# konstantineder/montecarlo-risk-engine

Hardware: AMD Instinct MI355X
Metric: path-steps/sec at 1M paths x 250 steps; PV/CVA rel-error vs CPU ref (higher is better)
Workload: dtype f64

## Files before the change

### montecarlo-risk-engine_amd/csrc/kf_lean.hip

```cpp
#include <cstdlib>
#include <map>
#include <utility>

#include "kf_common.h"

namespace {

template <int NSLOT, int PPL>
__device__ __forceinline__ void lean_date_cva(const FastDateCvaLds* __restrict__ rp, const double (&reg)[PPL][2 * NSLOT], double (&cva)[PPL],
                                              const double* __restrict__ etab)
{
    const mcx_expq_coef ec = mcx_expq_load(mcx_region_zero());
    const FastDateCvaLds r = *rp;
    double xe[2 * PPL], ev[2 * PPL];
#pragma unroll
    for (int q = 0; q < PPL; ++q) {
        xe[2 * q] = fma(r.m_s1, reg[q][FDC_S_REG], fma(r.m_n1, reg[q][FDC_NI_REG], r.m_c0));
        xe[2 * q + 1] = fma(r.c_c1, reg[q][FDC_C_REG], r.c_c0);
    }
    mcx_exp_tab_n<2 * PPL>(xe, ev, etab, ec);
#pragma unroll
    for (int q = 0; q < PPL; ++q) {
        const double x = fma(r.x_d, reg[q][FDC_X_REG], r.x_a);
        double p = 0.0;
        p += fma(fma(r.row0[2], x, r.row0[1]), x, r.row0[0]);
        p += fma(fma(r.row1[2], x, r.row1[1]), x, r.row1[0]);
        const double w = r.m_b * ev[2 * q];
        const double cs = fma(r.c_b, ev[2 * q + 1], r.c_a);
        cva[q] = fma(fmax(p, 0.0), w * (1.0 - cs), cva[q]);
    }
}

#define MCX_LEAN_WAVES 4
template <int NSLOT, int NZ, bool INJECT, int SIG, int PPL, bool SIMULATE, int DK = 0>
__global__ __launch_bounds__(MCX_BLOCK, MCX_LEAN_WAVES) void kf_lean(const FusedArgs)
{
    static_assert(DK == 0 || (SIG == SIG_VAS_CIR_E && SIMULATE && !INJECT), "the cva-date kernel simulates the Vasicek + CIR++ signature");
    constexpr int NREG = 2 * NSLOT;
    constexpr int TILE = MCX_BLOCK * PPL;
    extern __shared__ double lds[];
    KArgs& a0 = kargs_region(0);
    const int n_rec = a0.n_rec;
    const int64_t n = a0.k1.n;
    for (int q = threadIdx.x; q < 9 * n_rec; q += MCX_BLOCK) lds[q] = 0.0;
    FastDateCvaLds* const dlds = (FastDateCvaLds*)(lds + ((9 * n_rec + 1) & ~1));
    if constexpr (DK == 1) {
        const FastDateCva* __restrict__ dc = a0.cva_dates;
        const double* __restrict__ cf = a0.coeffs;
        const int n_dates = a0.n_dates;
        for (int q = threadIdx.x; q < 16 * n_dates; q += MCX_BLOCK) {
            const int t = q >> 4, e = q & 15;
            double v;
            if (e < FDC_HEAD) {
                v = ((const double*)(dc + t))[e];
            } else {
                const int off = e < FDC_HEAD + 3 ? dc[t].coeff_off0 : dc[t].coeff_off1;
                v = off >= 0 ? cf[off + (e - FDC_HEAD) % 3] : 0.0;
            }
            ((double*)dlds)[q] = v;
        }
    }
    constexpr int BMB = SIG == SIG_VAS_CIR_E ? 10 : 7;
    constexpr int BM = (INJECT || !SIMULATE) ? 0 : MCX_BM_LDS_DOUBLES_B(BMB);
    __shared__ double tab_lds[BM + MCX_EXP_LDS_DOUBLES];
    const double* tab = nullptr;
    const double* etab = tab_lds + BM;
    mcx_exp_tab_load(tab_lds + BM);
    if (BM) { mcx_bm_load<BMB>(tab_lds); tab = tab_lds; }
    __syncthreads();
    const int64_t tiles = (n + TILE - 1) / TILE;
    double n_block = 0.0;

    for (int64_t tile = blockIdx.x; tile < tiles; tile += gridDim.x) {
        const bool first_tile = tile == (int64_t)blockIdx.x;
        int64_t i[PPL];
        bool live[PPL];
        uint64_t path[PPL];
        double reg[PPL][NREG];
        double cfs[PPL], cva[PPL];
        int est[PPL];
        int n_init, n_steps;
        {
            KArgs& a = kargs_region(mcx_region_zero());
            const auto& k = a.k1;
#pragma unroll
            for (int q = 0; q < PPL; ++q) {
                const int64_t i_raw = tile * TILE + q * MCX_BLOCK + threadIdx.x;
                live[q] = i_raw < n;
                i[q] = live[q] ? i_raw : n - 1;
                path[q] = k.path_offset + (uint64_t)i[q];
                sim_init_state<NSLOT, SIG>(k, reg[q]);
                cfs[q] = 0.0; cva[q] = 0.0;
                est[q] = a.init_state[0];
            }
            const int64_t rest = n - tile * TILE;
            n_block += (double)(rest < TILE ? rest : TILE);
            n_init = k.n_initial_store; n_steps = k.n_steps;
        }
        if (SIMULATE) {
        int step = 0, t_init = 0;
#pragma unroll 1
        while (true) {
            const bool init = t_init < n_init;
            if (!init && step >= n_steps) break;
            int st = init ? t_init : -1;
            t_init += init ? 1 : 0;
            {
                const int zr0 = mcx_region_zero();
                const auto& k = kargs_region(zr0).k1;
                const uint64_t seed = k.seed;
                const mcx_bm_coef bc = mcx_bm_coef_load(zr0);
                const mcx_bm_vconst vc = mcx_bm_vconst_make<BMB>(bc);
#pragma unroll 1
                while (st < 0 && step < n_steps) {
                    if constexpr (SIG == SIG_GENERIC) {
#pragma unroll
                        for (int q = 0; q < PPL; ++q) sim_substep<NSLOT, NZ, INJECT, SIG, BMB, true>(k, step, path[q], i[q], reg[q], tab, seed, bc, &vc);
                        st = ldk(&k.steps[step].store_idx);
                    } else {
                        double zz[PPL][NZ], uu[PPL];
                        bool rare = false;
                        const StepData<NSLOT, NZ> sdat = sim_step_load<NSLOT, NZ, SIG>(k, step);
                        __builtin_amdgcn_sched_barrier(0);
                        if constexpr (INJECT) {
#pragma unroll
                            for (int q = 0; q < PPL; ++q) sim_draw<NZ, true, SIG, BMB>(k, step, path[q], i[q], zz[q], uu[q], tab, seed, bc, &vc);
                        } else {
                            uint32_t st_q[PPL];
#pragma unroll
                            for (int q = 0; q < PPL; ++q) st_q[q] = (uint32_t)step;
                            rare = sim_draw_n<PPL, NZ, SIG, BMB>(k, st_q, path, zz, uu, tab, seed, bc, vc);
                        }
                        if (!INJECT && __builtin_expect(__any(rare), 0)) {
#pragma unroll
                            for (int q = 0; q < PPL; ++q) sim_draw<NZ, false, SIG, BMB, true>(k, step, path[q], i[q], zz[q], uu[q], tab, seed, bc, &vc);
                        }
#pragma unroll
                        for (int q = 0; q < PPL; ++q) st = sim_apply_loaded<NSLOT, NZ, SIG, true>(k, sdat, reg[q], zz[q], uu[q]);
                    }
                    ++step;
                }
            }
            if (st >= 0) {
                if constexpr (DK == 1) lean_date_cva<NSLOT, PPL>(dlds + st, reg, cva, etab);
                else lean_date<NSLOT, SIG, PPL, true>(st, i, live, first_tile, lds, reg, cfs, cva, est, etab);
            }
        }
        } else {
            auto load_row = [&](int t, double (&dst)[PPL][NREG]) {
                const auto& k = kargs_region(0).k1;
                const int D = k.n_state;
#pragma unroll
                for (int q = 0; q < PPL; ++q)
#pragma unroll
                    for (int sl = 0; sl < NSLOT; ++sl) {
                        const bool bs = sig_kind(SIG, sl) >= 0 ? sig_is_bs(SIG, sl) : (k.slots[sl].kind == MCX_MODEL_BS);
                        const int c = k.slots[sl].state_off;
                        dst[q][2 * sl] = k.paths[((int64_t)t * D + c) * k.ld + i[q]];
                        dst[q][2 * sl + 1] = bs ? 0.0 : k.paths[((int64_t)t * D + c + 1) * k.ld + i[q]];
                    }
            };
            const int n_dates = kargs_region(0).n_dates;
            double bufb[PPL][NREG];
            load_row(0, reg);
            load_row(n_dates > 1 ? 1 : 0, bufb);
#pragma unroll 1
            for (int t = 0; t < n_dates; t += 2) {
                lean_date<NSLOT, SIG, PPL, false>(t, i, live, first_tile, lds, reg, cfs, cva, est, etab);
                if (t + 2 < n_dates) load_row(t + 2, reg);
                if (t + 1 < n_dates) {
                    lean_date<NSLOT, SIG, PPL, false>(t + 1, i, live, first_tile, lds, bufb, cfs, cva, est, etab);
                    if (t + 3 < n_dates) load_row(t + 3, bufb);
                }
            }
        }
        {
            KArgs& a = kargs_region(mcx_region_zero());
#pragma unroll
            for (int q = 0; q < PPL; ++q) if (a.cfs && live[q]) a.cfs[i[q]] = cfs[q];
            if (a.rec_pv[0] >= 0) lean_record<PPL>(cfs, live, a.rec_pv[0], n_rec, first_tile, lds);
            if (a.rec_cva[0] >= 0) {
                const double lgd = a.lgd[0];
                double cc[PPL];
#pragma unroll
                for (int q = 0; q < PPL; ++q) cc[q] = cva[q] * lgd;
                lean_record<PPL>(cc, live, a.rec_cva[0], n_rec, first_tile, lds);
            }
        }
    }
    __syncthreads();
    for (int r = threadIdx.x; r < n_rec; r += MCX_BLOCK) {
        double s1 = 0.0, s2 = 0.0;
        for (int w = 0; w < 4; ++w) { s1 += lds[n_rec + (w * n_rec + r) * 2]; s2 += lds[n_rec + (w * n_rec + r) * 2 + 1]; }
        double* dst = a0.partials + ((int64_t)blockIdx.x * n_rec + r) * 4;
        dst[0] = n_block; dst[1] = lds[r]; dst[2] = s1; dst[3] = s2;
    }
}

template <int NSLOT, int NZ, int SIG, int PPL>
int launch_lean_shape(const FusedArgs& a, int n_cu, bool inject, bool simulate, hipStream_t s)
{
    const int64_t tiles = (a.k1.n + MCX_BLOCK * PPL - 1) / (MCX_BLOCK * PPL);
    const size_t lds = sizeof(double) * (size_t)((9 * a.n_rec + 1) & ~1);
    const size_t lds_cva = lds + sizeof(FastDateCvaLds) * (size_t)a.n_dates;
    auto residency = [&](auto kernel, size_t bytes) {
        thread_local std::map<std::pair<const void*, size_t>, int> cache;
        const auto key = std::make_pair((const void*)kernel, bytes);
        auto it = cache.find(key);
        if (it == cache.end()) {
            int per_cu = 0;
            if (hipOccupancyMaxActiveBlocksPerMultiprocessor(&per_cu, kernel, MCX_BLOCK, bytes) != hipSuccess || per_cu < 1) per_cu = 1;
            it = cache.emplace(key, per_cu < MCX_LEAN_WAVES ? per_cu : MCX_LEAN_WAVES).first;
        }
        return (int64_t)it->second * n_cu;
    };
    auto sized = [&](int64_t resident) {
        if (tiles <= resident) return (int)tiles;
        const int64_t per = (tiles + resident - 1) / resident;
        return (int)((tiles + per - 1) / per);
    };
    int grid;
    if (!simulate) {
        auto kern = kf_lean<NSLOT, NZ, false, SIG, PPL, false>;
        grid = sized(residency(kern, lds));
        hipLaunchKernelGGL(kern, dim3(grid), dim3(MCX_BLOCK), lds, s, a);
    } else if (inject) {
        auto kern = kf_lean<NSLOT, NZ, true, SIG, PPL, true>;
        grid = sized(residency(kern, lds));
        hipLaunchKernelGGL(kern, dim3(grid), dim3(MCX_BLOCK), lds, s, a);
    } else {
        auto kern = kf_lean<NSLOT, NZ, false, SIG, PPL, true>;
        const int64_t resident = residency(kern, lds);
        if constexpr (SIG == SIG_VAS_CIR_E) {
            auto kern_cva = kf_lean<NSLOT, NZ, false, SIG, PPL, true, 1>;
            if (a.cva_dates && residency(kern_cva, lds_cva) >= resident) {
                grid = sized(resident);
                hipLaunchKernelGGL(kern_cva, dim3(grid), dim3(MCX_BLOCK), lds_cva, s, a);
                return grid;
            }
        }
        grid = sized(resident);
        hipLaunchKernelGGL(kern, dim3(grid), dim3(MCX_BLOCK), lds, s, a);
    }
    return grid;
}

template <int NSLOT, int NZ, int SIG>
void launch_lean(const FusedArgs& a, int n_cu, bool inject, bool simulate, hipStream_t s, int* grid_out)
{
    constexpr int PPL = (SIG == SIG_GENERIC && NSLOT >= 2) ? 1 : 2;
#ifdef MCX_LEAN_AB
    if (simulate && !inject) {
        const char* sh = getenv("MCX_LEAN_SHAPE");
        const int code = sh ? atoi(sh) : 0;
        if (code == 11) { *grid_out = launch_lean_shape<NSLOT, NZ, SIG, 1>(a, n_cu, inject, simulate, s); return; }
        if (code == 21) { *grid_out = launch_lean_shape<NSLOT, NZ, SIG, 2>(a, n_cu, inject, simulate, s); return; }
    }
#endif
    const int64_t full_tiles = (a.k1.n + MCX_BLOCK * PPL - 1) / (MCX_BLOCK * PPL);
    if (PPL == 2 && simulate && !inject && full_tiles < (int64_t)2 * n_cu) {
        *grid_out = launch_lean_shape<NSLOT, NZ, SIG, 1>(a, n_cu, inject, simulate, s);
        return;
    }
    *grid_out = launch_lean_shape<NSLOT, NZ, SIG, PPL>(a, n_cu, inject, simulate, s);
}

}

int mcx_launch_kf_lean(const FusedArgs& a, const mcx_sim_desc& sd, int n_cu, bool inject, bool simulate, hipStream_t s)
{
    int grid = -1;
    switch (mcx_sim_signature(sd)) {
    case SIG_VAS_CIR_E: launch_lean<2, 2, SIG_VAS_CIR_E>(a, n_cu, inject, simulate, s, &grid); break;
#ifndef MCX_LEAN_ONE_SIG
    case SIG_BS_A: launch_lean<1, 1, SIG_BS_A>(a, n_cu, inject, simulate, s, &grid); break;
    case SIG_BS_E: launch_lean<1, 1, SIG_BS_E>(a, n_cu, inject, simulate, s, &grid); break;
    case SIG_HESTON_QE: launch_lean<1, 2, SIG_HESTON_QE>(a, n_cu, inject, simulate, s, &grid); break;
    case SIG_HESTON_E: launch_lean<1, 2, SIG_HESTON_E>(a, n_cu, inject, simulate, s, &grid); break;
    case SIG_VAS_E: launch_lean<1, 1, SIG_VAS_E>(a, n_cu, inject, simulate, s, &grid); break;
    case SIG_VAS_A: launch_lean<1, 1, SIG_VAS_A>(a, n_cu, inject, simulate, s, &grid); break;
    case SIG_BS_VAS_CIRDET_E: launch_lean<3, 3, SIG_BS_VAS_CIRDET_E>(a, n_cu, inject, simulate, s, &grid); break;
    default:
        switch (sd.n_slots * 16 + sd.n_z) {
        case 1 * 16 + 1: launch_lean<1, 1, SIG_GENERIC>(a, n_cu, inject, simulate, s, &grid); break;
        case 1 * 16 + 2: launch_lean<1, 2, SIG_GENERIC>(a, n_cu, inject, simulate, s, &grid); break;
        case 2 * 16 + 2: launch_lean<2, 2, SIG_GENERIC>(a, n_cu, inject, simulate, s, &grid); break;
        case 3 * 16 + 3: launch_lean<3, 3, SIG_GENERIC>(a, n_cu, inject, simulate, s, &grid); break;
        case 4 * 16 + 4: launch_lean<4, 4, SIG_GENERIC>(a, n_cu, inject, simulate, s, &grid); break;
        default: break;
        }
#else
    default: break;
#endif
    }
    return grid;
}
```

### montecarlo-risk-engine_amd/csrc/mcx_device.h

```cpp
#pragma once
#include "mcx_internal.h"

struct K1Args {
    mcx_slot slots[MCX_MAX_SLOTS];
    double init_state[MCX_MAX_STATE];
    const mcx_step* __restrict__ steps;
    const double* __restrict__ chol;
    const double* __restrict__ aux;
    double* __restrict__ paths;
    const double* __restrict__ inject_z;
    const double* __restrict__ inject_u;
    const double* __restrict__ init_paths;
    int64_t n, ld;
    uint64_t seed, path_offset;
    int32_t scheme, n_steps, n_state, n_initial_store, flags, n_uniform;
};

static inline void mcx_fill_k1_args(const mcx_sim* sim, uint64_t seed, uint64_t path_offset, int64_t n_paths, int64_t ld,
                                    double* d_paths, const double* d_inject_z, const double* d_inject_u, K1Args* a)
{
    const mcx_sim_desc& d = sim->desc;
    memset(a, 0, sizeof(*a));
    for (int s = 0; s < d.n_slots; ++s) a->slots[s] = d.slots[s];
    for (int c = 0; c < d.n_state; ++c) a->init_state[c] = d.init_state[c];
    a->steps = sim->d_steps; a->chol = sim->d_chol; a->aux = sim->d_aux;
    a->paths = d_paths; a->inject_z = d_inject_z; a->inject_u = d_inject_u;
    a->n = n_paths; a->ld = ld; a->seed = seed; a->path_offset = path_offset;
    a->scheme = d.scheme; a->n_steps = d.n_steps; a->n_state = d.n_state; a->n_initial_store = d.n_initial_store;
    a->flags = d.flags; a->n_uniform = d.n_uniform;
}

__device__ __forceinline__ void philox4x32_10(uint32_t c0, uint32_t c1, uint32_t c2, uint32_t c3, uint32_t k0, uint32_t k1,
                                              uint32_t& o0, uint32_t& o1, uint32_t& o2, uint32_t& o3)
{
#pragma unroll
    for (int r = 0; r < 10; ++r) {
        const uint64_t p0 = (uint64_t)0xD2511F53u * c0;
        const uint64_t p1 = (uint64_t)0xCD9E8D57u * c2;
        const uint32_t n0 = __builtin_amdgcn_bitop3_b32((uint32_t)(p1 >> 32), c1, k0, 0x96);
        const uint32_t n2 = __builtin_amdgcn_bitop3_b32((uint32_t)(p0 >> 32), c3, k1, 0x96);
        c1 = (uint32_t)p1;
        c3 = (uint32_t)p0;
        c0 = n0;
        c2 = n2;
        k0 += 0x9E3779B9u;
        k1 += 0xBB67AE85u;
    }
    o0 = c0; o1 = c1; o2 = c2; o3 = c3;
}

__device__ __forceinline__ double u53(uint32_t lo, uint32_t hi, const mcx_bm_vconst* vc = nullptr)
{
    if (vc) return fma((double)hi, vc->s32, fma((double)(lo >> 11), vc->s53, vc->c54));
    return fma((double)hi, 0x1.0p-32, fma((double)(lo >> 11), 0x1.0p-53, 0x1.0p-54));
}

struct DevBridge {
    uint64_t seed, path_offset;
    const double* const* inject;
    int64_t ld;
};

__device__ __forceinline__ double dev_barrier_event(const DevEvent& e, const DevTerm* __restrict__ terms, const double* __restrict__ coeffs,
                                                    const DevBridge* __restrict__ bridge, const double* __restrict__ paths, int64_t D,
                                                    int64_t ld, int64_t i, double num)
{
    const int types = (int)e.aux[3];
    const int t1 = types & 7, t2 = types >> 3;
    const bool with_bridge = e.aux[0] == 5.0;
    double mx = -1.0e300, mn = 1.0e300, keep1 = 1.0, keep2 = 1.0, prev1 = 0.0, prev2 = 0.0;
    double c = 0.0;
    int draw_id = 0;
    DevBridge br = {0, 0, nullptr, 0};
    const double* __restrict__ inj = nullptr;
    if (with_bridge) {
        c = ldk(coeffs + e.coeff_off);
        draw_id = (int)ldk(coeffs + e.coeff_off + 1);
        br = ldk_struct(bridge);
        if (br.inject) inj = br.inject[draw_id];
    }
    AtomCache bc = {-1, -1, 0.0};
    for (int j = e.term_begin; j < e.term_end; ++j) {
        const double s = dev_atom_cached(ldk_struct(&terms[j]).atom, paths, D, ld, i, bc);
        mx = fmax(mx, s); mn = fmin(mn, s);
        if (with_bridge) {
            const double cur1 = mcx_log(s / e.aux[1]), cur2 = t2 ? mcx_log(s / e.aux[2]) : 0.0;
            if (j > e.term_begin) {
                const int k = j - e.term_begin - 1;
                for (int bi = 0; bi < (t2 ? 2 : 1); ++bi) {
                    const double p = mcx_exp(c * (bi ? prev2 * cur2 : prev1 * cur1));
                    double u;
                    if (inj) u = inj[(int64_t)(2 * k + bi) * br.ld + i];
                    else {
                        uint32_t w0, w1, w2, w3;
                        const uint64_t path = br.path_offset + (uint64_t)i;
                        philox4x32_10((uint32_t)path, (uint32_t)(path >> 32), (uint32_t)k, 0x80000000u | (uint32_t)(2 * draw_id + bi),
                                      (uint32_t)br.seed, (uint32_t)(br.seed >> 32), w0, w1, w2, w3);
                        u = u53(w0, w1);
                    }
                    const double hit = fmin(fmax((p - u + 0.05) / 0.1, 0.0), 1.0);
                    if (bi) keep2 *= 1.0 - hit; else keep1 *= 1.0 - hit;
                }
            }
            prev1 = cur1; prev2 = cur2;
        }
    }
    double pay = fmax(e.sign * (dev_atom(e.x, paths, D, ld, i) - e.strike), 0.0) * dev_barrier_ind(t1, e.aux[1], mx, mn);
    if (with_bridge) pay *= (t1 <= 2) ? keep1 : 1.0 - keep1;
    if (t2) {
        pay *= dev_barrier_ind(t2, e.aux[2], mx, mn);
        if (with_bridge) pay *= (t2 <= 2) ? keep2 : 1.0 - keep2;
    }
    return pay / num;
}

template <bool TAB = false, int BMB = 7, bool GUARD = true>
__device__ __forceinline__ bool pair_from_words(uint32_t w0, uint32_t w1, uint32_t w2, uint32_t w3, double& ua, double& z0, double& z1,
                                                const double* __restrict__ tab, const mcx_bm_coef& bc, const mcx_bm_vconst* vc = nullptr)
{
    ua = u53(w0, w1, vc);
    double s, c, r;
    if (TAB) {
        const double r2 = mcx_m2log_tab<BMB>(ua, tab, bc, vc);
        if (!GUARD) r = mcx_sqrt_gp(r2);
        else if (__builtin_expect(__any(w1 == 0xffffffffu), 0)) r = ua < 1.0 ? mcx_sqrt_g(r2) : 0.0;
        else r = mcx_sqrt_gp(r2);
        const int j = (int)(w3 >> (32 - BMB));
        const double ur = u53(w2, w3 & ((1u << (32 - BMB)) - 1u), vc);
        mcx_sincos2pi_tab<BMB>(ur, j, tab, s, c, bc, vc);
    } else {
        r = mcx_sqrt(-2.0 * mcx_log(ua));
        mcx_sincos2pi(u53(w2, w3), s, c);
    }
    z0 = r * c;
    z1 = r * s;
    return w1 == 0xffffffffu;
}

template <bool TAB = false, int BMB = 7, bool GUARD = true>
__device__ __forceinline__ bool draw_pair(uint64_t seed, uint64_t path, uint32_t step, uint32_t draw, double& ua, double& z0, double& z1,
                                          const double* __restrict__ tab, const mcx_bm_coef& bc, const mcx_bm_vconst* vc = nullptr)
{
    uint32_t w0, w1, w2, w3;
    philox4x32_10((uint32_t)path, (uint32_t)(path >> 32), step, draw, (uint32_t)seed, (uint32_t)(seed >> 32), w0, w1, w2, w3);
    return pair_from_words<TAB, BMB, GUARD>(w0, w1, w2, w3, ua, z0, z1, tab, bc, vc);
}

template <bool TAB = false>
__device__ __forceinline__ void draw_pair(uint64_t seed, uint64_t path, uint32_t step, uint32_t draw, double& ua, double& z0, double& z1,
                                          const double* __restrict__ tab = nullptr)
{
    const mcx_bm_coef bc = mcx_bm_coef_load();
    draw_pair<TAB>(seed, path, step, draw, ua, z0, z1, tab, bc);
}

__device__ __forceinline__ double degree_of_truth(double x, bool fuzzy, double eps)
{
    if (!fuzzy) return x > 0.0 ? 1.0 : 0.0;
    const double v = (x + eps) / (2.0 * eps);
    return fmin(fmax(v, 0.0), 1.0);
}

struct AuxPtr {
    const double* __restrict__ p;
    __device__ __forceinline__ double operator[](int i) const { return ldk(p + i); }
    __device__ __forceinline__ mcx_aux_drv drv() const { return ldk_struct((const mcx_aux_drv*)(p + MCX_AUX_C0)); }
};
struct AuxRegs {
    double v[MCX_AUX];
    __device__ __forceinline__ double operator[](int i) const { return v[i]; }
    __device__ __forceinline__ mcx_aux_drv drv() const { mcx_aux_drv d; d.c0 = v[MCX_AUX_C0]; d.c1 = v[MCX_AUX_C1]; d.c2 = v[MCX_AUX_C2]; return d; }
};

template <int KIND, int SCHEME, bool POS = false, class SL, class AUX>
__device__ __forceinline__ void step_slot(const SL& sl, int scheme_rt, int flags, double dt, double sq,
                                          const AUX& aux, double& s0, double& s1, double zc0, double zc1, double u)
{
    const auto* p = sl.p;
    const int scheme = SCHEME >= 0 ? SCHEME : scheme_rt;
    switch (KIND >= 0 ? KIND : sl.kind) {
    case MCX_MODEL_BS:
        if (scheme == MCX_SCHEME_ANALYTICAL) {
            s0 = s0 * mcx_exp(aux[0] + (zc0 - aux[1]));
        } else {
            const mcx_aux_drv dc = aux.drv();
            s0 = fma(s0, fma(dc.c2, zc0, dc.c0), s0);
        }
        break;
    case MCX_MODEL_VASICEK: {
        const double r = s0;
        s1 = s1 + r * dt;
        if (scheme == MCX_SCHEME_ANALYTICAL) s0 = (p[2] + (r - p[2]) * aux[0]) + zc0;
        else {
            const mcx_aux_drv dc = aux.drv();
            s0 = fma(dc.c1, r, s0);
            s0 = fma(dc.c2, zc0, s0);
            s0 = s0 + dc.c0;
        }
        break;
    }
    case MCX_MODEL_HW: {
        const double r = s0;
        s1 = s1 + r * dt;
        if (scheme == MCX_SCHEME_ANALYTICAL) s0 = r * aux[0] + aux[1] + zc0;
        else s0 = r + (aux[0] - p[3] * r) * dt + p[1] * sq * zc0;
        break;
    }
    case MCX_MODEL_CIRPP: {
        const double y = s0;
        const double sy = POS ? mcx_sqrt_gp(y) : mcx_sqrt_g(y);
        const mcx_aux_drv dc = aux.drv();
        s1 = fma(y + aux[0], dt, s1);
        s0 = fma(dc.c1, y, s0);
        s0 = fma(dc.c2 * sy, zc0, s0);
        s0 = s0 + dc.c0;
        s0 = fmax(s0, 1e-12);
        break;
    }
    case MCX_MODEL_CIRPP_DET:
        s1 = s1 + aux[0] * dt;
        s0 = aux[1];
        break;
    case MCX_MODEL_S2F: {
        const double x = s0, y = s1;
        if (scheme == MCX_SCHEME_ANALYTICAL) {
            s0 = x * aux[0] + zc0;
            s1 = y + p[3] * dt + zc1;
        } else {
            s0 = x - p[1] * x * dt + p[2] * sq * zc0;
            s1 = y + p[3] * dt + p[4] * sq * zc1;
        }
        break;
    }
    case MCX_MODEL_HESTON: {
        const double logS = s0, v = s1;
        const double sigma = p[1], rate = p[2], kappa = p[4], theta = p[5];
        if (scheme == MCX_SCHEME_EULER) {
            const double sv = mcx_sqrt(fmax(v, 0.0));
            s0 = logS + (rate - 0.5 * v) * dt + sv * sq * zc0;
            s1 = fmax(v + kappa * (theta - v) * dt + sigma * sv * sq * zc1, 0.0);
        } else {
            const double eps = 1e-12;
            const bool fuzzy = (flags & MCX_FLAG_SMOOTHING) != 0;
            const double m = theta + (v - theta) * aux[0];
            const double s2 = v * aux[6] + aux[7];
            const double omu = fmax(1.0 - u, eps);
            const double d1 = m * m + eps, d5 = m + eps;
            const double d15 = d1 * d5;
            const double ra = mcx_rcp(d15 * omu);
            const double r_omu = ra * d15, ra6 = ra * omu;
            const double r1 = ra6 * d5, r5 = ra6 * d1;
            const double psi = s2 * r1;
            const double d2 = psi + eps, d4 = psi + 1.0;
            const double rb = mcx_rcp(d2 * d4);
            const double invpsi = rb * d4, r4 = rb * d2;
            const double t = fmax(2.0 * invpsi - 1.0, 0.0);
            double root = mcx_sqrt_g(2.0 * invpsi * t);
            root = invpsi < 0.0 ? __builtin_nan("") : root;
            const double b2u = 2.0 * invpsi - 1.0 + root;
            const double b2 = b2u < 0.0 ? 0.0 : b2u;
            const double b = mcx_sqrt_g(b2);
            const double pp = fmin(fmax((psi - 1.0) * r4, 0.0), 1.0 - 1e-6);
            const double beta = (1.0 - pp) * r5;
            const double d3 = 1.0 + b2, d7 = beta + eps;
            const double rc = mcx_rcp(d3 * d7);
            const double a = m * (rc * d7);
            const double v1 = a * (b + zc1) * (b + zc1);
            const double omp = fmax(1.0 - pp, eps);
            const double v_tail = mcx_log(omp * r_omu) * (rc * d3);
            const double v2 = degree_of_truth(u - pp, fuzzy, 0.3) * v_tail;
            const double w = degree_of_truth(psi - 1.5, fuzzy, 0.5);
            const double vn = (1.0 - w) * v1 + w * v2;
            const double var_int = fmax(aux[4] * v + aux[5] * vn, 0.0);
            const double vol = mcx_sqrt_gp(fmax(var_int, eps));
            s0 = logS + rate * dt + aux[1] + aux[2] * v + aux[3] * vn + vol * zc0;
            s1 = vn;
        }
        break;
    }
    default: break;
    }
}


enum { SIG_GENERIC = 0, SIG_VAS_CIR_E = 1, SIG_BS_A = 2, SIG_BS_E = 3, SIG_HESTON_QE = 4, SIG_HESTON_E = 5,
       SIG_VAS_E = 6, SIG_VAS_A = 7, SIG_BS_VAS_CIRDET_E = 8 };

__host__ __device__ constexpr int sig_kind(int sig, int slot)
{
    return sig == SIG_VAS_CIR_E ? (slot == 0 ? MCX_MODEL_VASICEK : MCX_MODEL_CIRPP)
         : (sig == SIG_BS_A || sig == SIG_BS_E) ? MCX_MODEL_BS
         : (sig == SIG_HESTON_QE || sig == SIG_HESTON_E) ? MCX_MODEL_HESTON
         : (sig == SIG_VAS_E || sig == SIG_VAS_A) ? MCX_MODEL_VASICEK
         : sig == SIG_BS_VAS_CIRDET_E ? (slot == 0 ? MCX_MODEL_BS : slot == 1 ? MCX_MODEL_VASICEK : MCX_MODEL_CIRPP_DET)
         : -1;
}
__host__ __device__ constexpr int sig_scheme(int sig)
{
    return (sig == SIG_VAS_CIR_E || sig == SIG_BS_E || sig == SIG_HESTON_E || sig == SIG_VAS_E || sig == SIG_BS_VAS_CIRDET_E) ? MCX_SCHEME_EULER
         : (sig == SIG_BS_A || sig == SIG_VAS_A) ? MCX_SCHEME_ANALYTICAL
         : sig == SIG_HESTON_QE ? MCX_SCHEME_QE : -1;
}
__host__ __device__ constexpr bool sig_is_bs(int sig, int slot) { return sig_kind(sig, slot) == MCX_MODEL_BS; }

static inline int mcx_sim_signature(const mcx_sim_desc& d)
{
    auto k = [&](int s) { return d.slots[s].kind; };
    if (d.n_slots == 2 && k(0) == MCX_MODEL_VASICEK && k(1) == MCX_MODEL_CIRPP && d.scheme == MCX_SCHEME_EULER) return SIG_VAS_CIR_E;
    if (d.n_slots == 3 && k(0) == MCX_MODEL_BS && k(1) == MCX_MODEL_VASICEK && k(2) == MCX_MODEL_CIRPP_DET && d.scheme == MCX_SCHEME_EULER)
        return SIG_BS_VAS_CIRDET_E;
    if (d.n_slots == 1) {
        if (k(0) == MCX_MODEL_BS) return d.scheme == MCX_SCHEME_ANALYTICAL ? SIG_BS_A : d.scheme == MCX_SCHEME_EULER ? SIG_BS_E : SIG_GENERIC;
        if (k(0) == MCX_MODEL_HESTON) return d.scheme == MCX_SCHEME_QE ? SIG_HESTON_QE : d.scheme == MCX_SCHEME_EULER ? SIG_HESTON_E : SIG_GENERIC;
        if (k(0) == MCX_MODEL_VASICEK) return d.scheme == MCX_SCHEME_EULER ? SIG_VAS_E : d.scheme == MCX_SCHEME_ANALYTICAL ? SIG_VAS_A : SIG_GENERIC;
    }
    return SIG_GENERIC;
}

__device__ __forceinline__ AuxPtr aux_of_slot(const double* __restrict__ ax, int s) { return AuxPtr{ax + s * MCX_AUX}; }
template <int NSLOT>
__device__ __forceinline__ const AuxRegs& aux_of_slot(const AuxRegs (&ax)[NSLOT], int s) { return ax[s]; }

template <int NSLOT, int NZ, int SIG, int S, bool POS = false, class KA, class AX>
__device__ __forceinline__ void step_slots(const KA& k, const mcx_step& sp, const AX& ax,
                                           double (&reg)[2 * NSLOT], const double (&zc)[NZ], double u)
{
    if constexpr (S < NSLOT) {
        const double zc0 = (NSLOT == 1) ? zc[0] : zc[S < NZ ? S : 0];
        const double zc1 = (NSLOT == 1 && NZ > 1) ? zc[NZ > 1 ? 1 : 0] : 0.0;
        step_slot<sig_kind(SIG, S), sig_scheme(SIG), POS>(k.slots[S], k.scheme, k.flags | k.slots[S].flags, sp.dt, sp.sqrt_dt,
                                                      aux_of_slot(ax, S), reg[2 * S], reg[2 * S + 1], zc0, zc1, u);
        step_slots<NSLOT, NZ, SIG, S + 1, POS>(k, sp, ax, reg, zc, u);
    }
}

template <int NZ, bool INJECT, int SIG, int BMB = 7, bool GUARD = true, class KA>
__device__ __forceinline__ bool sim_draw(const KA& k, int step, uint64_t path, int64_t i, double (&z)[NZ], double& u,
                                         const double* __restrict__ tab, uint64_t seed, const mcx_bm_coef& bc, const mcx_bm_vconst* vc = nullptr)
{
    u = 0.0;
    bool rare = false;
    if (INJECT) {
#pragma unroll
        for (int j = 0; j < NZ; ++j) z[j] = k.inject_z[((int64_t)step * NZ + j) * k.ld + i];
        if (k.n_uniform) u = k.inject_u[(int64_t)step * k.ld + i];
    } else {
        double ua;
#pragma unroll
        for (int q = 0; q < (NZ + 1) / 2; ++q) {
            double z0, z1;
            rare |= draw_pair<true, BMB, GUARD>(seed, path, (uint32_t)step, (uint32_t)q, ua, z0, z1, tab, bc, vc);
            z[2 * q] = z0;
            if (2 * q + 1 < NZ) z[2 * q + 1] = z1;
        }
        if (sig_scheme(SIG) == MCX_SCHEME_QE || (sig_scheme(SIG) < 0 && k.n_uniform)) {
            double z0, z1;
            draw_pair<false>(seed, path, (uint32_t)step, (uint32_t)((NZ + 1) / 2), u, z0, z1, nullptr, bc);
        }
    }
    return rare;
}

template <int PPL>
__device__ __forceinline__ void philox4x32_10_n(const uint64_t (&path)[PPL], const uint32_t (&step)[PPL], uint32_t draw, uint64_t seed,
                                                uint32_t (&o0)[PPL], uint32_t (&o1)[PPL], uint32_t (&o2)[PPL], uint32_t (&o3)[PPL])
{
    uint32_t c0[PPL], c1[PPL], c2[PPL], c3[PPL];
#pragma unroll
    for (int q = 0; q < PPL; ++q) { c0[q] = (uint32_t)path[q]; c1[q] = (uint32_t)(path[q] >> 32); c2[q] = step[q]; c3[q] = draw; }
    uint32_t k0 = (uint32_t)seed, k1 = (uint32_t)(seed >> 32);
#pragma unroll
    for (int r = 0; r < 10; ++r) {
#pragma unroll
        for (int q = 0; q < PPL; ++q) {
            const uint64_t p0 = (uint64_t)0xD2511F53u * c0[q];
            const uint64_t p1 = (uint64_t)0xCD9E8D57u * c2[q];
            const uint32_t n0 = __builtin_amdgcn_bitop3_b32((uint32_t)(p1 >> 32), c1[q], k0, 0x96);
            const uint32_t n2 = __builtin_amdgcn_bitop3_b32((uint32_t)(p0 >> 32), c3[q], k1, 0x96);
            c1[q] = (uint32_t)p1; c3[q] = (uint32_t)p0; c0[q] = n0; c2[q] = n2;
        }
        k0 += 0x9E3779B9u;
        k1 += 0xBB67AE85u;
    }
#pragma unroll
    for (int q = 0; q < PPL; ++q) { o0[q] = c0[q]; o1[q] = c1[q]; o2[q] = c2[q]; o3[q] = c3[q]; }
}

template <int PPL, int BMB>
__device__ __forceinline__ bool draw_pairs_staged(uint64_t seed, const uint64_t (&path)[PPL], const uint32_t (&step)[PPL], uint32_t draw,
                                                  double (&z0)[PPL], double (&z1)[PPL], const double* __restrict__ tab,
                                                  const mcx_bm_coef& C, const mcx_bm_vconst& vc)
{
    constexpr int N = 1 << BMB, LOG_TERMS = mcx_bm_shape<BMB>::LOG_TERMS;
    uint32_t w0[PPL], w1[PPL], w2[PPL], w3[PPL];
    philox4x32_10_n<PPL>(path, step, draw, seed, w0, w1, w2, w3);
    double m[PPL], ed[PPL], ps[PPL], pc[PPL];
    int e[PPL];
    mcx_d2 tc[PPL], sc[PPL];
#pragma unroll
    for (int q = 0; q < PPL; ++q) {
        const double ua = u53(w0[q], w1[q], &vc);
        m[q] = __builtin_amdgcn_frexp_mant(ua);
        e[q] = __builtin_amdgcn_frexp_exp(ua);
        const int jl = (__double2hiint(m[q]) >> (20 - BMB)) & (N - 1);
        tc[q] = ((const mcx_d2*)tab)[jl];
        sc[q] = ((const mcx_d2*)(tab + 2 * N))[(int)(w3[q] >> (32 - BMB))];
    }
    __builtin_amdgcn_sched_barrier(0);
#pragma unroll
    for (int q = 0; q < PPL; ++q) {
        const double ur = u53(w2[q], w3[q] & ((1u << (32 - BMB)) - 1u), &vc);
        const double d = fma(ur, 6.28318530717958647692, vc.trig_off);
        const double d2 = d * d;
        double qs, qc;
        if constexpr (mcx_bm_shape<BMB>::TRIG_TERMS == 3) {
            qs = fma(fma(vc.sin_head, d2, C.c[7]), d2, C.c[6]);
            qc = fma(fma(vc.cos_head, d2, C.c[10]), d2, C.c[9]);
        } else {
            qs = fma(vc.sin_head, d2, C.c[6]);
            qc = fma(vc.cos_head, d2, C.c[9]);
        }
        ps[q] = fma(d * d2, qs, d);
        pc[q] = fma(d2, qc, 1.0);
        ed[q] = (double)e[q];
    }
    __builtin_amdgcn_sched_barrier(0);
    bool rare = false;
#pragma unroll
    for (int q = 0; q < PPL; ++q) {
        const double s = fma(m[q], tc[q].x, 2.0);
        double p = vc.log_head;
#pragma unroll
        for (int k = LOG_TERMS - 2; k >= 0; --k) p = fma(p, s, C.c[k]);
        const double r2 = fma(ed[q], -2.0 * 6.93147180559945309417e-01, tc[q].y) + fma(s * s, p, s);
        const double r = mcx_sqrt_gp(r2);
        const double sn = fma(sc[q].x, pc[q], sc[q].y * ps[q]);
        const double cs = fma(-sc[q].x, ps[q], sc[q].y * pc[q]);
        z0[q] = r * cs;
        z1[q] = r * sn;
        rare |= w1[q] == 0xffffffffu;
    }
    return rare;
}

template <int PPL, int NZ, int SIG, int BMB, class KA>
__device__ __forceinline__ bool sim_draw_n(const KA& k, const uint32_t (&step)[PPL], const uint64_t (&path)[PPL], double (&z)[PPL][NZ], double (&u)[PPL],
                                           const double* __restrict__ tab, uint64_t seed, const mcx_bm_coef& bc, const mcx_bm_vconst& vc)
{
    bool rare = false;
#pragma unroll
    for (int dq = 0; dq < (NZ + 1) / 2; ++dq) {
        double a[PPL], b[PPL];
        rare |= draw_pairs_staged<PPL, BMB>(seed, path, step, (uint32_t)dq, a, b, tab, bc, vc);
#pragma unroll
        for (int q = 0; q < PPL; ++q) { z[q][2 * dq] = a[q]; if (2 * dq + 1 < NZ) z[q][2 * dq + 1] = b[q]; }
    }
#pragma unroll
    for (int q = 0; q < PPL; ++q) {
        u[q] = 0.0;
        if (sig_scheme(SIG) == MCX_SCHEME_QE || (sig_scheme(SIG) < 0 && k.n_uniform)) {
            double t0, t1;
            draw_pair<false>(seed, path[q], step[q], (uint32_t)((NZ + 1) / 2), u[q], t0, t1, nullptr, bc);
        }
    }
    return rare;
}

template <int NSLOT, int NZ, int SIG, bool POS = false, class KA>
__device__ __forceinline__ int sim_apply(const KA& k, int step, double (&reg)[2 * NSLOT], const double (&z)[NZ], double u)
{
    const mcx_step sp = ldk_struct(&k.steps[step]);
    double zc[NZ];
    constexpr bool UNIT_L00 = sig_scheme(SIG) == MCX_SCHEME_EULER || sig_scheme(SIG) == MCX_SCHEME_QE;
    const double* __restrict__ L = UNIT_L00 ? k.chol : k.chol + (int64_t)sp.chol_idx * NZ * NZ;
#pragma unroll
    for (int r = 0; r < NZ; ++r) {
        double acc = (UNIT_L00 && r == 0) ? z[0] : ldk(L + r * NZ) * z[0];
#pragma unroll
        for (int c = 1; c <= r; ++c) acc = fma(ldk(L + r * NZ + c), z[c], acc);
        zc[r] = acc;
    }
    const double* __restrict__ ax = k.aux + (int64_t)step * NSLOT * MCX_AUX;
    step_slots<NSLOT, NZ, SIG, 0, POS>(k, sp, ax, reg, zc, u);
    return sp.store_idx;
}

template <int NSLOT, int NZ>
struct StepData {
    mcx_step sp;
    double L[NZ * NZ];
    AuxRegs ax[NSLOT];
};
template <int NSLOT, int NZ, int SIG, class KA>
__device__ __forceinline__ StepData<NSLOT, NZ> sim_step_load(const KA& k, int step)
{
    StepData<NSLOT, NZ> d;
    d.sp = ldk_struct(&k.steps[step]);
    constexpr bool UNIT_L00 = sig_scheme(SIG) == MCX_SCHEME_EULER || sig_scheme(SIG) == MCX_SCHEME_QE;
    const double* __restrict__ L = UNIT_L00 ? k.chol : k.chol + (int64_t)d.sp.chol_idx * NZ * NZ;
#pragma unroll
    for (int q = 0; q < NZ * NZ; ++q) d.L[q] = ldk(L + q);
    struct P2 { double v[2]; };
    struct P4 { double v[4]; };
    static_assert(MCX_AUX == 8, "aux row layout");
    const double* __restrict__ ax = k.aux + (int64_t)step * NSLOT * MCX_AUX;
#pragma unroll
    for (int s = 0; s < NSLOT; ++s) {
        const P2 a = ldk_struct((const P2*)(ax + s * MCX_AUX)), b = ldk_struct((const P2*)(ax + s * MCX_AUX + 2));
        const P4 c = ldk_struct((const P4*)(ax + s * MCX_AUX + 4));
        d.ax[s].v[0] = a.v[0]; d.ax[s].v[1] = a.v[1]; d.ax[s].v[2] = b.v[0]; d.ax[s].v[3] = b.v[1];
#pragma unroll
        for (int q = 0; q < 4; ++q) d.ax[s].v[4 + q] = c.v[q];
    }
    return d;
}
template <int NSLOT, int NZ, int SIG, bool POS = false, class KA>
__device__ __forceinline__ int sim_apply_loaded(const KA& k, const StepData<NSLOT, NZ>& d, double (&reg)[2 * NSLOT], const double (&z)[NZ], double u)
{
    double zc[NZ];
    constexpr bool UNIT_L00 = sig_scheme(SIG) == MCX_SCHEME_EULER || sig_scheme(SIG) == MCX_SCHEME_QE;
#pragma unroll
    for (int r = 0; r < NZ; ++r) {
        double acc = (UNIT_L00 && r == 0) ? z[0] : d.L[r * NZ] * z[0];
#pragma unroll
        for (int c = 1; c <= r; ++c) acc = fma(d.L[r * NZ + c], z[c], acc);
        zc[r] = acc;
    }
    step_slots<NSLOT, NZ, SIG, 0, POS>(k, d.sp, d.ax, reg, zc, u);
    return d.sp.store_idx;
}

template <int NSLOT, int NZ, bool INJECT, int SIG, int BMB = 7, bool POS = false, class KA>
__device__ __forceinline__ void sim_substep(const KA& k, int step, uint64_t path, int64_t i, double (&reg)[2 * NSLOT],
                                            const double* __restrict__ tab, uint64_t seed, const mcx_bm_coef& bc, const mcx_bm_vconst* vc = nullptr)
{
    double z[NZ], u;
    sim_draw<NZ, INJECT, SIG, BMB>(k, step, path, i, z, u, tab, seed, bc, vc);
    sim_apply<NSLOT, NZ, SIG, POS>(k, step, reg, z, u);
}

__host__ __device__ constexpr int mcx_kind_state_dim(int kind) { return kind == MCX_MODEL_BS ? 1 : kind == MCX_MODEL_S2F ? 3 : 2; }

template <int NSLOT, int SIG, class KA>
__device__ __forceinline__ void sim_init_state(const KA& k, double (&reg)[2 * NSLOT], int64_t i = 0)
{
    const double* __restrict__ ip = k.init_paths;
#pragma unroll
    for (int s = 0; s < NSLOT; ++s) {
        const int kind = sig_kind(SIG, s) >= 0 ? sig_kind(SIG, s) : k.slots[s].kind;
        const int c = k.slots[s].state_off + (kind == MCX_MODEL_S2F ? 1 : 0);
        if (ip) {
            reg[2 * s] = ip[(int64_t)c * k.ld + i];
            reg[2 * s + 1] = kind == MCX_MODEL_BS ? 0.0 : ip[(int64_t)(c + 1) * k.ld + i];
        } else {
            reg[2 * s] = k.init_state[c];
            reg[2 * s + 1] = kind == MCX_MODEL_BS ? 0.0 : k.init_state[c + 1];
        }
    }
}

template <int NSLOT, int SIG, class KA>
__device__ __forceinline__ void sim_store_state(const KA& k, int t, int64_t i, const double (&reg)[2 * NSLOT],
                                                const double* __restrict__ ax = nullptr)
{
    const int D = k.n_state;
#pragma unroll
    for (int s = 0; s < NSLOT; ++s) {
        const int kind = sig_kind(SIG, s) >= 0 ? sig_kind(SIG, s) : k.slots[s].kind;
        const int c = k.slots[s].state_off;
        if (kind == MCX_MODEL_S2F) {
            const double logF = ax ? ldk(ax + s * MCX_AUX + 1) : k.slots[s].p[6];
            double logS = (logF + reg[2 * s]) + reg[2 * s + 1];
            if (!ax && k.init_paths) logS = k.init_paths[(int64_t)c * k.ld + i];
            k.paths[((int64_t)t * D + c) * k.ld + i] = logS;
            k.paths[((int64_t)t * D + c + 1) * k.ld + i] = reg[2 * s];
            k.paths[((int64_t)t * D + c + 2) * k.ld + i] = reg[2 * s + 1];
            continue;
        }
        k.paths[((int64_t)t * D + c) * k.ld + i] = reg[2 * s];
        if (kind != MCX_MODEL_BS) k.paths[((int64_t)t * D + c + 1) * k.ld + i] = reg[2 * s + 1];
    }
}
```

Baseline: 291.8 billion.

## Specialise Philox first rounds for uniform path high word and stop after last live CVA date

When every path in the launch shares the same upper 32 bits of the path index, a UHI kernel variant is selected. It partly evaluates the first three Philox rounds, using the known zero high counter word and the wave-uniform high bits, which removes a few multiplies and xors per draw. Separately, the CVA-date kernel scans the date table for the last date with nonzero regression coefficients and ends simulation once that date is processed, skipping the remaining steps. This adds template instantiations and host-side selection logic. The early exit assumes dates whose coefficients are all zero contribute nothing to CVA.

```diff
diff --git a/montecarlo-risk-engine_amd/csrc/kf_lean.hip b/montecarlo-risk-engine_amd/csrc/kf_lean.hip
--- a/montecarlo-risk-engine_amd/csrc/kf_lean.hip
+++ b/montecarlo-risk-engine_amd/csrc/kf_lean.hip
@@ -32,10 +32,11 @@
 }
 
 #define MCX_LEAN_WAVES 4
-template <int NSLOT, int NZ, bool INJECT, int SIG, int PPL, bool SIMULATE, int DK = 0>
+template <int NSLOT, int NZ, bool INJECT, int SIG, int PPL, bool SIMULATE, int DK = 0, bool UHI = false>
 __global__ __launch_bounds__(MCX_BLOCK, MCX_LEAN_WAVES) void kf_lean(const FusedArgs)
 {
     static_assert(DK == 0 || (SIG == SIG_VAS_CIR_E && SIMULATE && !INJECT), "the cva-date kernel simulates the Vasicek + CIR++ signature");
+    static_assert(!UHI || (SIG != SIG_GENERIC && SIMULATE && !INJECT), "the uniform high word is for the kernels that draw through sim_draw_n");
     constexpr int NREG = 2 * NSLOT;
     constexpr int TILE = MCX_BLOCK * PPL;
     extern __shared__ double lds[];
@@ -68,6 +69,17 @@
     mcx_exp_tab_load(tab_lds + BM);
     if (BM) { mcx_bm_load<BMB>(tab_lds); tab = tab_lds; }
     __syncthreads();
+    int t_last = -1;
+    if constexpr (DK == 1) {
+        for (int t = a0.n_dates - 1; t >= 0 && t_last < 0; --t) {
+            const FastDateCvaLds* r = dlds + t;
+            bool nz = false;
+#pragma unroll
+            for (int e = 0; e < 3; ++e) nz |= (r->row0[e] != 0.0) | (r->row1[e] != 0.0);
+            if (nz) t_last = t;
+        }
+        t_last = __builtin_amdgcn_readfirstlane(t_last);
+    }
     const int64_t tiles = (n + TILE - 1) / TILE;
     double n_block = 0.0;
 
@@ -99,8 +111,12 @@
         }
         if (SIMULATE) {
         int step = 0, t_init = 0;
+        int t_done = -1;
 #pragma unroll 1
         while (true) {
+#ifndef MCX_LEAN_NO_LIVE_DATE
+            if (DK == 1 && t_done >= t_last) break;
+#endif
             const bool init = t_init < n_init;
             if (!init && step >= n_steps) break;
             int st = init ? t_init : -1;
@@ -109,6 +125,7 @@
                 const int zr0 = mcx_region_zero();
                 const auto& k = kargs_region(zr0).k1;
                 const uint64_t seed = k.seed;
+                const uint32_t path_hi = UHI ? (uint32_t)(k.path_offset >> 32) : 0u;
                 const mcx_bm_coef bc = mcx_bm_coef_load(zr0);
                 const mcx_bm_vconst vc = mcx_bm_vconst_make<BMB>(bc);
 #pragma unroll 1
@@ -129,7 +146,7 @@
                             uint32_t st_q[PPL];
 #pragma unroll
                             for (int q = 0; q < PPL; ++q) st_q[q] = (uint32_t)step;
-                            rare = sim_draw_n<PPL, NZ, SIG, BMB>(k, st_q, path, zz, uu, tab, seed, bc, vc);
+                            rare = sim_draw_n<PPL, NZ, SIG, BMB, UHI>(k, st_q, path, zz, uu, tab, seed, bc, vc, path_hi);
                         }
                         if (!INJECT && __builtin_expect(__any(rare), 0)) {
 #pragma unroll
@@ -142,7 +159,7 @@
                 }
             }
             if (st >= 0) {
-                if constexpr (DK == 1) lean_date_cva<NSLOT, PPL>(dlds + st, reg, cva, etab);
+                if constexpr (DK == 1) { lean_date_cva<NSLOT, PPL>(dlds + st, reg, cva, etab); t_done = st; }
                 else lean_date<NSLOT, SIG, PPL, true>(st, i, live, first_tile, lds, reg, cfs, cva, est, etab);
             }
         }
@@ -229,10 +246,17 @@
         grid = sized(residency(kern, lds));
         hipLaunchKernelGGL(kern, dim3(grid), dim3(MCX_BLOCK), lds, s, a);
     } else {
-        auto kern = kf_lean<NSLOT, NZ, false, SIG, PPL, true>;
+#ifdef MCX_LEAN_NO_UHI
+        constexpr bool HAS_UHI = false;
+#else
+        constexpr bool HAS_UHI = SIG != SIG_GENERIC;
+#endif
+        const uint64_t p_first = a.k1.path_offset, p_last = p_first + (uint64_t)a.k1.n - 1;
+        const bool uhi = HAS_UHI && a.k1.n > 0 && (p_first >> 32) == (p_last >> 32);
+        auto kern = uhi ? kf_lean<NSLOT, NZ, false, SIG, PPL, true, 0, HAS_UHI> : kf_lean<NSLOT, NZ, false, SIG, PPL, true>;
         const int64_t resident = residency(kern, lds);
         if constexpr (SIG == SIG_VAS_CIR_E) {
-            auto kern_cva = kf_lean<NSLOT, NZ, false, SIG, PPL, true, 1>;
+            auto kern_cva = uhi ? kf_lean<NSLOT, NZ, false, SIG, PPL, true, 1, HAS_UHI> : kf_lean<NSLOT, NZ, false, SIG, PPL, true, 1>;
             if (a.cva_dates && residency(kern_cva, lds_cva) >= resident) {
                 grid = sized(resident);
                 hipLaunchKernelGGL(kern_cva, dim3(grid), dim3(MCX_BLOCK), lds_cva, s, a);
diff --git a/montecarlo-risk-engine_amd/csrc/mcx_device.h b/montecarlo-risk-engine_amd/csrc/mcx_device.h
--- a/montecarlo-risk-engine_amd/csrc/mcx_device.h
+++ b/montecarlo-risk-engine_amd/csrc/mcx_device.h
@@ -361,16 +361,47 @@
     return rare;
 }
 
-template <int PPL>
+template <int PPL, bool UHI = false>
 __device__ __forceinline__ void philox4x32_10_n(const uint64_t (&path)[PPL], const uint32_t (&step)[PPL], uint32_t draw, uint64_t seed,
-                                                uint32_t (&o0)[PPL], uint32_t (&o1)[PPL], uint32_t (&o2)[PPL], uint32_t (&o3)[PPL])
-{
+                                                uint32_t (&o0)[PPL], uint32_t (&o1)[PPL], uint32_t (&o2)[PPL], uint32_t (&o3)[PPL],
+                                                uint32_t hi = 0)
+{
+    constexpr uint32_t M0 = 0xD2511F53u, M1 = 0xCD9E8D57u, W0 = 0x9E3779B9u, W1 = 0xBB67AE85u;
     uint32_t c0[PPL], c1[PPL], c2[PPL], c3[PPL];
-#pragma unroll
-    for (int q = 0; q < PPL; ++q) { c0[q] = (uint32_t)path[q]; c1[q] = (uint32_t)(path[q] >> 32); c2[q] = step[q]; c3[q] = draw; }
     uint32_t k0 = (uint32_t)seed, k1 = (uint32_t)(seed >> 32);
-#pragma unroll
-    for (int r = 0; r < 10; ++r) {
+    if constexpr (UHI) {
+        uint32_t c3s[PPL];
+#pragma unroll
+        for (int q = 0; q < PPL; ++q) {
+            const uint64_t s1 = (uint64_t)M1 * step[q];
+            const uint32_t n0 = (uint32_t)(s1 >> 32) ^ hi ^ k0;
+            const uint64_t v0 = (uint64_t)M0 * (uint32_t)path[q];
+            const uint32_t n2 = (uint32_t)(v0 >> 32) ^ (draw ^ k1);
+            const uint64_t s0 = (uint64_t)M0 * n0;
+            const uint64_t v1 = (uint64_t)M1 * n2;
+            c0[q] = (uint32_t)(v1 >> 32) ^ ((uint32_t)s1 ^ (k0 + W0));
+            c2[q] = (uint32_t)v0 ^ ((uint32_t)(s0 >> 32) ^ (k1 + W1));
+            c1[q] = (uint32_t)v1;
+            c3s[q] = (uint32_t)s0;
+        }
+        k0 += 2 * W0;
+        k1 += 2 * W1;
+#pragma unroll
+        for (int q = 0; q < PPL; ++q) {
+            const uint64_t p0 = (uint64_t)M0 * c0[q];
+            const uint64_t p1 = (uint64_t)M1 * c2[q];
+            const uint32_t n0 = __builtin_amdgcn_bitop3_b32((uint32_t)(p1 >> 32), c1[q], k0, 0x96);
+            const uint32_t n2 = (uint32_t)(p0 >> 32) ^ (c3s[q] ^ k1);
+            c1[q] = (uint32_t)p1; c3[q] = (uint32_t)p0; c0[q] = n0; c2[q] = n2;
+        }
+        k0 += W0;
+        k1 += W1;
+    } else {
+#pragma unroll
+        for (int q = 0; q < PPL; ++q) { c0[q] = (uint32_t)path[q]; c1[q] = (uint32_t)(path[q] >> 32); c2[q] = step[q]; c3[q] = draw; }
+    }
+#pragma unroll
+    for (int r = UHI ? 3 : 0; r < 10; ++r) {
 #pragma unroll
         for (int q = 0; q < PPL; ++q) {
             const uint64_t p0 = (uint64_t)0xD2511F53u * c0[q];
@@ -386,14 +417,14 @@
     for (int q = 0; q < PPL; ++q) { o0[q] = c0[q]; o1[q] = c1[q]; o2[q] = c2[q]; o3[q] = c3[q]; }
 }
 
-template <int PPL, int BMB>
+template <int PPL, int BMB, bool UHI = false>
 __device__ __forceinline__ bool draw_pairs_staged(uint64_t seed, const uint64_t (&path)[PPL], const uint32_t (&step)[PPL], uint32_t draw,
                                                   double (&z0)[PPL], double (&z1)[PPL], const double* __restrict__ tab,
-                                                  const mcx_bm_coef& C, const mcx_bm_vconst& vc)
+                                                  const mcx_bm_coef& C, const mcx_bm_vconst& vc, uint32_t hi = 0)
 {
     constexpr int N = 1 << BMB, LOG_TERMS = mcx_bm_shape<BMB>::LOG_TERMS;
     uint32_t w0[PPL], w1[PPL], w2[PPL], w3[PPL];
-    philox4x32_10_n<PPL>(path, step, draw, seed, w0, w1, w2, w3);
+    philox4x32_10_n<PPL, UHI>(path, step, draw, seed, w0, w1, w2, w3, hi);
     double m[PPL], ed[PPL], ps[PPL], pc[PPL];
     int e[PPL];
     mcx_d2 tc[PPL], sc[PPL];
@@ -443,15 +474,16 @@
     return rare;
 }
 
-template <int PPL, int NZ, int SIG, int BMB, class KA>
+template <int PPL, int NZ, int SIG, int BMB, bool UHI = false, class KA>
 __device__ __forceinline__ bool sim_draw_n(const KA& k, const uint32_t (&step)[PPL], const uint64_t (&path)[PPL], double (&z)[PPL][NZ], double (&u)[PPL],
-                                           const double* __restrict__ tab, uint64_t seed, const mcx_bm_coef& bc, const mcx_bm_vconst& vc)
+                                           const double* __restrict__ tab, uint64_t seed, const mcx_bm_coef& bc, const mcx_bm_vconst& vc,
+                                           uint32_t hi = 0)
 {
     bool rare = false;
 #pragma unroll
     for (int dq = 0; dq < (NZ + 1) / 2; ++dq) {
         double a[PPL], b[PPL];
-        rare |= draw_pairs_staged<PPL, BMB>(seed, path, step, (uint32_t)dq, a, b, tab, bc, vc);
+        rare |= draw_pairs_staged<PPL, BMB, UHI>(seed, path, step, (uint32_t)dq, a, b, tab, bc, vc, hi);
 #pragma unroll
         for (int q = 0; q < PPL; ++q) { z[q][2 * dq] = a[q]; if (2 * dq + 1 < NZ) z[q][2 * dq + 1] = b[q]; }
     }
```

After: 302.1 billion, median of 6. 3.5% higher.
